# RLHF-V/RLAIF-V

Hardware: NVIDIA B200
Metric: preference-pairs/sec LLaVA-1.5-7B DPO step (higher is better)
Workload: dtype bf16

## Files before the change

### include/rlaifv_b200.h

```cpp
#ifndef RLAIFV_B200_H_
#define RLAIFV_B200_H_

#ifdef __cplusplus
extern "C" {
#endif

const char* rlaifv_last_error(void);

int rlaifv_gemm_bf16(const void* A, long long lda, int a_mn_major, const void* B, long long ldb,
                     int b_mn_major, void* C, long long ldc, int M, int N, int K, const void* bias,
                     const void* residual, long long ldr, int act, int accumulate, int tile_n,
                     void* stream);

int rlaifv_gemm_bf16_scaled(const void* A, long long lda, int a_mn_major, const void* B, long long ldb,
                            int b_mn_major, void* C, long long ldc, int M, int N, int K, const void* bias,
                            const void* residual, long long ldr, int act, int accumulate, int tile_n, float alpha,
                            void* stream);

int rlaifv_gemm_bf16_dual(const void* A, long long lda, int a_mn_major, const void* B, long long ldb, int b_mn_major,
                          const void* A2, long long lda2, const void* B2, long long ldb2, int K2, int r, int n_sub,
                          void* C, long long ldc, int M, int N, int K, const void* bias, const void* residual,
                          long long ldr, int act, int accumulate, void* stream);

int rlaifv_gemm_bf16_swiglu_bwd(const void* A, long long lda, const void* B, long long ldb, int b_mn_major,
// ... 21 lines not shown
                         long long ld_out, const void* d_out, long long ld_dout, const float* lse,
                         float* dq_f32, void* dk, void* dv, long long ld_dkv, float* delta_ws, int nseq,
                         int S, int n_heads, int head_dim, float scale, void* stream);

int rlaifv_attention_fwd_gqa(const void* q, const void* k, const void* v, long long ld_qkv, void* out,
                             long long ld_out, float* lse, int nseq, int S, int n_heads, int n_kv_heads,
                             int head_dim, int causal, float scale, void* stream);
int rlaifv_attention_bwd_gqa(const void* q, const void* k, const void* v, long long ld_qkv, const void* out,
                             long long ld_out, const void* d_out, long long ld_dout, const float* lse, float* dq_f32,
                             void* dk, void* dv, long long ld_dkv, float* delta_ws, int nseq, int S, int n_heads,
                             int n_kv_heads, int head_dim, float scale, void* stream);
int rlaifv_cross_attention_fwd(const void* q, long long ld_q, const void* k, const void* v, long long ld_kv, void* out,
                               long long ld_out, float* lse, int nseq, int Sq, int Skv, int n_heads, int head_dim,
                               int q_shared, float scale, void* stream);
int rlaifv_cross_attention_bwd(const void* q, long long ld_q, const void* k, const void* v, long long ld_kv,
                               const void* out, long long ld_out, const void* d_out, long long ld_dout,
                               const float* lse, float* dq_f32, void* dk, void* dv, long long ld_dkv, float* delta_ws,
                               int nseq, int Sq, int Skv, int n_heads, int head_dim, int q_shared, float scale,
                               void* stream);
int rlaifv_rope_fwd_gqa(void* qkv, const void* cos_tab, const void* sin_tab, long long M, int T, int n_heads,
                        int n_kv_heads, int head_dim, long long ld, void* stream);
int rlaifv_rope_bwd_gqa(void* dqkv, const float* dq_f32, const void* cos_tab, const void* sin_tab, long long M,
                        int T, int n_heads, int n_kv_heads, int head_dim, long long ld, void* stream);

int rlaifv_rmsnorm_fwd(const void* x, const void* w, void* y, float* rstd_or_null, int M, int H, float eps,
                       void* stream);
int rlaifv_rmsnorm_bwd_partials(void);
int rlaifv_rmsnorm_bwd(const void* dy, const void* x, const void* w, const float* rstd,
                       const void* dres_or_null, void* dx, void* dw, int dw_accumulate, float* workspace,
                       int M, int H, void* stream);
int rlaifv_layernorm_fwd(const void* x, const void* w, const void* b, void* y, int M, int H, float eps,
                         void* stream);
int rlaifv_layernorm_bwd(const void* dy, const void* x, const void* w, void* dx, void* dw, void* db, int accumulate,
                         float* workspace, int M, int H, float eps, void* stream);
int rlaifv_add_rows_bcast(const void* x, const void* table, void* y, long long M, int P, int H, void* stream);

int rlaifv_rope_fwd(void* qkv, const void* cos_tab, const void* sin_tab, long long M, int T, int n_heads,
                    int head_dim, long long ld, void* stream);
int rlaifv_rope_bwd(void* dqkv, const float* dq_f32, const void* cos_tab, const void* sin_tab, long long M,
                    int T, int n_heads, int head_dim, long long ld, void* stream);

int rlaifv_swiglu_fwd(const void* gu, void* act, long long M, int F, void* stream);
int rlaifv_swiglu_bwd(const void* gu, const void* dact, void* dgu, long long M, int F, void* stream);
int rlaifv_gelu_fwd(const void* pre, void* post, long long n, void* stream);
int rlaifv_gelu_bwd(const void* pre, const void* dpost, void* dpre, long long n, void* stream);
int rlaifv_colsum(const void* x, long long M, int N, void* db, int accumulate, float* workspace_64xN,
// ... 62 lines not shown
```

### rlaif-v_b200/csrc/rowops.cu

```cuda
#include "common.cuh"
#include "host_util.h"

namespace b200 {

__device__ __forceinline__ void load8(const bf16* p, float (&v)[8]) {
  uint4 u = *reinterpret_cast<const uint4*>(p);
  float2 a = unpack_bf16(u.x), b = unpack_bf16(u.y), c = unpack_bf16(u.z), d = unpack_bf16(u.w);
  v[0] = a.x; v[1] = a.y; v[2] = b.x; v[3] = b.y; v[4] = c.x; v[5] = c.y; v[6] = d.x; v[7] = d.y;
}
__device__ __forceinline__ void store8(bf16* p, const float (&v)[8]) {
  uint4 u;
  u.x = pack_bf16(v[0], v[1]);
  u.y = pack_bf16(v[2], v[3]);
  u.z = pack_bf16(v[4], v[5]);
  u.w = pack_bf16(v[6], v[7]);
  *reinterpret_cast<uint4*>(p) = u;
}

__device__ __forceinline__ float2 block_sum2(float a, float b) {
  __shared__ float sa[32], sb[32];
  a = warp_sum(a);
  b = warp_sum(b);
  const int w = threadIdx.x >> 5, l = threadIdx.x & 31, nw = blockDim.x >> 5;
  __syncthreads();
// ... 334 lines not shown
    const long long row = r / nrot;
    const int pos = (int)(row % T);
    bf16* p = dqkv + row * ld + (long long)head * D + c8 * 8;
    float y1[8], y2[8], c1[8], s1[8], c2[8], s2[8];
    if (head < nh && dq_f32) {
      const float* q = dq_f32 + row * (long long)nh * D + head * D + c8 * 8;
      float4 a = *reinterpret_cast<const float4*>(q), b = *reinterpret_cast<const float4*>(q + 4);
      float4 c = *reinterpret_cast<const float4*>(q + half), d = *reinterpret_cast<const float4*>(q + half + 4);
      y1[0] = a.x; y1[1] = a.y; y1[2] = a.z; y1[3] = a.w; y1[4] = b.x; y1[5] = b.y; y1[6] = b.z; y1[7] = b.w;
      y2[0] = c.x; y2[1] = c.y; y2[2] = c.z; y2[3] = c.w; y2[4] = d.x; y2[5] = d.y; y2[6] = d.z; y2[7] = d.w;
    } else {
      load8(p, y1);
      load8(p + half, y2);
    }
    load8(cosb + (long long)pos * D + c8 * 8, c1);
    load8(sinb + (long long)pos * D + c8 * 8, s1);
    load8(cosb + (long long)pos * D + half + c8 * 8, c2);
    load8(sinb + (long long)pos * D + half + c8 * 8, s2);
    float o1[8], o2[8];
#pragma unroll
    for (int j = 0; j < 8; ++j) {
      o1[j] = y1[j] * c1[j] + y2[j] * s2[j];
      o2[j] = y2[j] * c2[j] - y1[j] * s1[j];
    }
    store8(p, o1);
    store8(p + half, o2);
  }
}

__global__ void swiglu_fwd_kernel(const bf16* __restrict__ gu, bf16* __restrict__ act, long long M,
                                  int F) {
  const int nch = F >> 3;
  const long long total = M * nch;
  const long long T = (long long)gridDim.x * blockDim.x;
  for (long long idx = (long long)blockIdx.x * blockDim.x + threadIdx.x; idx < total; idx += 2 * T) {
    const long long idx2 = idx + T;
    const bool two = idx2 < total;
    const long long row0 = idx / nch, row1 = two ? idx2 / nch : row0;
    const int c0 = (int)(idx - row0 * nch), c1 = two ? (int)(idx2 - row1 * nch) : c0;
    float g0[8], u0[8], g1[8], u1[8], o[8];
    load8(gu + row0 * 2 * F + c0 * 8, g0);
    load8(gu + row0 * 2 * F + F + c0 * 8, u0);
    load8(gu + row1 * 2 * F + c1 * 8, g1);
    load8(gu + row1 * 2 * F + F + c1 * 8, u1);
#pragma unroll
    for (int j = 0; j < 8; ++j) o[j] = bf16_round(g0[j] / (1.f + __expf(-g0[j]))) * u0[j];
// ... 747 lines not shown
  const long long total = M * (n_heads + n_kv_heads) * (head_dim / 16);
  rope_bwd_kernel<<<grid_for(total, 256), 256, 0, ST>>>((bf16*)dqkv, dq_f32, (const bf16*)cos_tab,
                                                        (const bf16*)sin_tab, M, T, n_heads, n_kv_heads, head_dim, ld);
  B200_CHECK_CUDA(cudaGetLastError());
  return 0;
}
extern "C" int rlaifv_rope_fwd(void* qkv, const void* cos_tab, const void* sin_tab, long long M, int T,
                               int n_heads, int head_dim, long long ld, void* stream) {
  return rope_fwd_impl(qkv, cos_tab, sin_tab, M, T, n_heads, n_heads, head_dim, ld, stream);
}
extern "C" int rlaifv_rope_bwd(void* dqkv, const float* dq_f32, const void* cos_tab, const void* sin_tab,
                               long long M, int T, int n_heads, int head_dim, long long ld, void* stream) {
  return rope_bwd_impl(dqkv, dq_f32, cos_tab, sin_tab, M, T, n_heads, n_heads, head_dim, ld, stream);
}
extern "C" int rlaifv_rope_fwd_gqa(void* qkv, const void* cos_tab, const void* sin_tab, long long M, int T,
                                   int n_heads, int n_kv_heads, int head_dim, long long ld, void* stream) {
  return rope_fwd_impl(qkv, cos_tab, sin_tab, M, T, n_heads, n_kv_heads, head_dim, ld, stream);
}
extern "C" int rlaifv_rope_bwd_gqa(void* dqkv, const float* dq_f32, const void* cos_tab, const void* sin_tab,
                                   long long M, int T, int n_heads, int n_kv_heads, int head_dim, long long ld,
                                   void* stream) {
  return rope_bwd_impl(dqkv, dq_f32, cos_tab, sin_tab, M, T, n_heads, n_kv_heads, head_dim, ld, stream);
}

extern "C" int rlaifv_swiglu_fwd(const void* gu, void* act, long long M, int F, void* stream) {
  B200_REQUIRE(F % 8 == 0, "swiglu: F %% 8 != 0");
  swiglu_fwd_kernel<<<grid_for(M * (F / 8), 256), 256, 0, ST>>>((const bf16*)gu, (bf16*)act, M, F);
  B200_CHECK_CUDA(cudaGetLastError());
  return 0;
}
extern "C" int rlaifv_swiglu_bwd(const void* gu, const void* dact, void* dgu, long long M, int F, void* stream) {
  B200_REQUIRE(F % 8 == 0, "swiglu: F %% 8 != 0");
  swiglu_bwd_kernel<<<grid_for(M * (F / 8), 256), 256, 0, ST>>>((const bf16*)gu, (const bf16*)dact, (bf16*)dgu, M, F);
  B200_CHECK_CUDA(cudaGetLastError());
  return 0;
}
extern "C" int rlaifv_gelu_fwd(const void* pre, void* post, long long n, void* stream) {
  B200_REQUIRE(n % 8 == 0, "gelu_fwd: n %% 8 != 0");
  gelu_fwd_kernel<<<grid_for(n / 8, 256), 256, 0, ST>>>((const bf16*)pre, (bf16*)post, n / 8);
  B200_CHECK_CUDA(cudaGetLastError());
  return 0;
}
extern "C" int rlaifv_gelu_bwd(const void* pre, const void* dpost, void* dpre, long long n, void* stream) {
  B200_REQUIRE(n % 8 == 0, "gelu_bwd: n %% 8 != 0");
  gelu_bwd_kernel<<<grid_for(n / 8, 256), 256, 0, ST>>>((const bf16*)pre, (const bf16*)dpost, (bf16*)dpre, n / 8);
  B200_CHECK_CUDA(cudaGetLastError());
// ... 111 lines not shown
  splice_token_weight_kernel<<<grid_for((long long)nseq * (T - 1), 256), 256, 0, ST>>>(src, token_weight, out, nseq, Lw, T);
  B200_CHECK_CUDA(cudaGetLastError());
  return 0;
}
extern "C" int rlaifv_supervised_rows(const long long* labels, int nseq, int T, int cap, int* row_pos, void* stream) {
  B200_REQUIRE(nseq > 0 && T >= 2 && cap > 0, "supervised_rows: bad shape");
  B200_REQUIRE((long long)nseq * T < 2147483647LL, "supervised_rows: nseq*T overflows int32");
  supervised_rows_kernel<<<nseq, 32, 0, ST>>>(labels, nseq, T, cap, row_pos);
  B200_CHECK_CUDA(cudaGetLastError());
  return 0;
}
extern "C" int rlaifv_rows_gather(const int* row_pos, const void* x, void* out, long long n_rows, int H, void* stream) {
  B200_REQUIRE(H % 8 == 0 && n_rows > 0, "rows_gather: bad shape");
  rows_gather_kernel<<<grid_for(n_rows * (H / 8), 256), 256, 0, ST>>>(row_pos, (const bf16*)x, (bf16*)out, n_rows, H / 8);
  B200_CHECK_CUDA(cudaGetLastError());
  return 0;
}
extern "C" int rlaifv_rows_scatter(const int* row_pos, const void* dy, void* dx, long long n_rows, int H, void* stream) {
  B200_REQUIRE(H % 8 == 0 && n_rows > 0, "rows_scatter: bad shape");
  rows_scatter_kernel<<<grid_for(n_rows * (H / 8), 256), 256, 0, ST>>>(row_pos, (const bf16*)dy, (bf16*)dx, n_rows, H / 8);
  B200_CHECK_CUDA(cudaGetLastError());
  return 0;
}
extern "C" int rlaifv_logp_fwd_rows(const void* logits, long long ld, const long long* labels, const int* row_pos,
                                    long long n_rows, int nseq, int T, int V, float* per_tok, float* lse,
                                    float* logp_sum, float* logp_avg, float* count, void* stream) {
  B200_REQUIRE(V % 8 == 0 && T >= 2 && n_rows > 0 && row_pos, "logp_fwd_rows: bad arguments");
  const int grid = (int)(n_rows < (long long)num_sms() * 8 ? n_rows : (long long)num_sms() * 8);
  logp_fwd_kernel<<<grid, LOGP_THREADS, 0, ST>>>((const bf16*)logits, ld, labels, nseq, T, V, per_tok, lse, row_pos,
                                                 n_rows);
  B200_CHECK_CUDA(cudaGetLastError());
  logp_reduce_kernel<<<nseq, 256, 0, ST>>>(per_tok, labels, nseq, T, logp_sum, logp_avg, count);
  B200_CHECK_CUDA(cudaGetLastError());
  return 0;
}
extern "C" int rlaifv_logp_bwd_rows(void* logits, long long ld, const long long* labels, const int* row_pos,
                                    long long n_rows, const float* lse, const float* d_logp, const float* token_weight,
                                    const float* norm, int nseq, int T, int V, void* stream) {
  B200_REQUIRE(V % 8 == 0 && n_rows > 0 && row_pos, "logp_bwd_rows: bad arguments");
  const int grid = (int)(n_rows < (long long)num_sms() * 8 ? n_rows : (long long)num_sms() * 8);
  logp_bwd_weighted_kernel<<<grid, LOGP_THREADS, 0, ST>>>((bf16*)logits, ld, labels, lse, d_logp, token_weight, norm,
                                                          nseq, T, V, row_pos, n_rows);
  B200_CHECK_CUDA(cudaGetLastError());
  return 0;
}
extern "C" int rlaifv_logp_bwd(void* logits, long long ld, const long long* labels, const float* lse,
// ... 81 lines not shown
```

### rlaif-v_b200/lib.py

```python
import ctypes
import os

import torch

_HERE = os.path.dirname(os.path.abspath(__file__))
LIB_PATH = os.path.join(_HERE, "librlaifv_b200.so")

c_void_p = ctypes.c_void_p
c_int = ctypes.c_int
c_ll = ctypes.c_longlong
c_float = ctypes.c_float

_SIGNATURES = {
    "rlaifv_gemm_bf16": [c_void_p, c_ll, c_int, c_void_p, c_ll, c_int, c_void_p, c_ll, c_int, c_int, c_int,
                         c_void_p, c_void_p, c_ll, c_int, c_int, c_int, c_void_p],
    "rlaifv_gemm_bf16_scaled": [c_void_p, c_ll, c_int, c_void_p, c_ll, c_int, c_void_p, c_ll, c_int, c_int, c_int,
                                c_void_p, c_void_p, c_ll, c_int, c_int, c_int, c_float, c_void_p],
    "rlaifv_gemm_bf16_dual": [c_void_p, c_ll, c_int, c_void_p, c_ll, c_int, c_void_p, c_ll, c_void_p, c_ll, c_int, c_int,
                              c_int, c_void_p, c_ll, c_int, c_int, c_int, c_void_p, c_void_p, c_ll, c_int, c_int,
                              c_void_p],
    "rlaifv_gemm_bf16_swiglu_bwd": [c_void_p, c_ll, c_void_p, c_ll, c_int, c_void_p, c_ll, c_void_p, c_ll, c_int, c_void_p,
                                    c_ll, c_void_p, c_ll, c_int, c_int, c_int, c_void_p],
    "rlaifv_gemm_set_2cta": [c_int],
    "rlaifv_attention_set_variant": [c_int],
# ... 12 lines not shown
    "rlaifv_swiglu_fwd": [c_void_p, c_void_p, c_ll, c_int, c_void_p],
    "rlaifv_swiglu_bwd": [c_void_p, c_void_p, c_void_p, c_ll, c_int, c_void_p],
    "rlaifv_gelu_fwd": [c_void_p, c_void_p, c_ll, c_void_p],
    "rlaifv_gelu_bwd": [c_void_p, c_void_p, c_void_p, c_ll, c_void_p],
    "rlaifv_dropout_fwd": [c_void_p, c_void_p, c_ll, c_float, ctypes.c_ulonglong, c_void_p],
    "rlaifv_dropout_bwd_add": [c_void_p, c_void_p, c_ll, c_float, ctypes.c_ulonglong, c_void_p],
    "rlaifv_colsum": [c_void_p, c_ll, c_int, c_void_p, c_int, c_void_p, c_void_p],
    "rlaifv_clip_im2col": [c_void_p, c_void_p, c_int, c_int, c_int, c_int, c_int, c_void_p],
    "rlaifv_clip_embed": [c_void_p, c_void_p, c_void_p, c_void_p, c_int, c_int, c_int, c_void_p],
    "rlaifv_clip_drop_cls": [c_void_p, c_void_p, c_int, c_int, c_int, c_void_p],
    "rlaifv_splice_count": [c_void_p, c_int, c_int, c_int, c_int, c_void_p, c_void_p, c_void_p],
    "rlaifv_splice_map": [c_void_p, c_void_p, c_void_p, c_void_p, c_int, c_int, c_int, c_int, c_int,
                          c_void_p, c_void_p, c_void_p],
    "rlaifv_splice_gather": [c_void_p, c_void_p, c_void_p, c_void_p, c_void_p, c_int, c_int, c_int, c_int,
                             c_void_p],
    "rlaifv_splice_scatter": [c_void_p, c_void_p, c_void_p, c_void_p, c_void_p, c_int, c_int, c_int, c_int,
                              c_void_p],
    "rlaifv_f32_to_bf16": [c_void_p, c_void_p, c_ll, c_int, c_void_p],
    "rlaifv_f32_to_bf16_2d": [c_void_p, c_ll, c_void_p, c_ll, c_ll, c_int, c_int, c_void_p],
    "rlaifv_splice_token_weight": [c_void_p, c_void_p, c_void_p, c_int, c_int, c_int, c_void_p],
    "rlaifv_supervised_rows": [c_void_p, c_int, c_int, c_int, c_void_p, c_void_p],
    "rlaifv_rows_gather": [c_void_p, c_void_p, c_void_p, c_ll, c_int, c_void_p],
    "rlaifv_rows_scatter": [c_void_p, c_void_p, c_void_p, c_ll, c_int, c_void_p],
    "rlaifv_logp_fwd_rows": [c_void_p, c_ll, c_void_p, c_void_p, c_ll, c_int, c_int, c_int, c_void_p, c_void_p, c_void_p,
                             c_void_p, c_void_p, c_void_p],
    "rlaifv_logp_bwd_rows": [c_void_p, c_ll, c_void_p, c_void_p, c_ll, c_void_p, c_void_p, c_void_p, c_void_p, c_int,
                             c_int, c_int, c_void_p],
    "rlaifv_logp_fwd": [c_void_p, c_ll, c_void_p, c_int, c_int, c_int, c_void_p, c_void_p, c_void_p,
                        c_void_p, c_void_p, c_void_p],
    "rlaifv_logp_bwd": [c_void_p, c_ll, c_void_p, c_void_p, c_void_p, c_void_p, c_int, c_int, c_int,
                        c_void_p],
    "rlaifv_dpo_loss": [c_void_p, c_void_p, c_void_p, c_void_p, c_int, c_float, c_float, c_float, c_float,
                        c_void_p, c_void_p, c_void_p, c_void_p, c_void_p, c_void_p, c_void_p],
    "rlaifv_adamw_step": [c_void_p, c_void_p, c_void_p, c_void_p, c_int, c_void_p, c_ll, c_float, c_float,
                          c_float, c_float, c_float, c_int, c_float, c_void_p],
    "rlaifv_attention_fwd_gqa": [c_void_p, c_void_p, c_void_p, c_ll, c_void_p, c_ll, c_void_p, c_int, c_int,
                                 c_int, c_int, c_int, c_int, c_float, c_void_p],
    "rlaifv_attention_bwd_gqa": [c_void_p, c_void_p, c_void_p, c_ll, c_void_p, c_ll, c_void_p, c_ll, c_void_p,
                                 c_void_p, c_void_p, c_void_p, c_ll, c_void_p, c_int, c_int, c_int, c_int, c_int,
                                 c_float, c_void_p],
    "rlaifv_rope_fwd_gqa": [c_void_p, c_void_p, c_void_p, c_ll, c_int, c_int, c_int, c_int, c_ll, c_void_p],
    "rlaifv_rope_bwd_gqa": [c_void_p, c_void_p, c_void_p, c_void_p, c_ll, c_int, c_int, c_int, c_int, c_ll, c_void_p],
    "rlaifv_attention_fwd": [c_void_p, c_void_p, c_void_p, c_ll, c_void_p, c_ll, c_void_p, c_int, c_int,
                             c_int, c_int, c_int, c_float, c_void_p],
    "rlaifv_attention_bwd": [c_void_p, c_void_p, c_void_p, c_ll, c_void_p, c_ll, c_void_p, c_ll, c_void_p,
                             c_void_p, c_void_p, c_void_p, c_ll, c_void_p, c_int, c_int, c_int, c_int,
# ... 117 lines not shown
```

### rlaif-v_b200/model.py

```python
import math
from dataclasses import dataclass, field

import torch

from . import ops

IGNORE_INDEX = -100
IMAGE_TOKEN_INDEX = -200
_BF = torch.bfloat16
_F32 = torch.float32


@dataclass
class LlavaDims:
    vocab_size: int = 32000
    hidden_size: int = 4096
    intermediate_size: int = 11008
    num_layers: int = 32
    num_heads: int = 32
    num_kv_heads: int = 0
    rms_eps: float = 1e-5
    rope_theta: float = 10000.0
    max_len: int = 2048
    clip_hidden: int = 1024
# ... 22 lines not shown
    @property
    def kv_size(self):
        return self.kv_heads * self.head_dim

    @property
    def num_patches(self):
        return (self.image_size // self.patch_size) ** 2

    @property
    def clip_layers_used(self):
        return self.clip_layers + 1 + self.select_layer if self.select_layer < 0 else self.select_layer

    @property
    def patch_k(self):
        return 3 * self.patch_size * self.patch_size

    @property
    def patch_k_pad(self):
        return (self.patch_k + 63) // 64 * 64


def _round_up(n, m):
    return (n + m - 1) // m * m


@dataclass
class Segment:
    name: str
    shape: tuple
    offset: int
    decay: bool


@dataclass
class Bucket:
    name: str
    start: int
    size: int
    decay_size: int
    segments: list = field(default_factory=list)


class ParamStore:
    PAD = 1024

    def __init__(self, dims: LlavaDims, device):
# ... 208 lines not shown
            self.layers.append(L)


class LlavaDPOPolicy:

    def __init__(self, dims: LlavaDims, device="cuda", hf_state=None, seed=0, init_std=0.02):
        self.dims = dims
        self.device = torch.device(device)
        self.store = ParamStore(dims, self.device)
        has_clip = dims.frontend == "clip_mlp"
        if hf_state is not None:
            self.store.load_hf(hf_state)
            self.clip = ClipWeights(dims, self.device, hf_state) if has_clip else None
        else:
            self._random_init(seed, init_std)
            self.clip = ClipWeights(dims, self.device, None, seed + 1) if has_clip else None
        self._rope = {}
        self._bufs = {}
        self.stash_extra = False
        self.stash_act = False
        self.compact_head = True
        self.split_attention_bwd = True
        self.fuse_swiglu_bwd = True
        self.embed_grad_f32 = None
        self._stash = None
        self.lora = None

    def enable_lora(self, r=64, alpha=16, seed=7, init_b_zero=True, dropout=0.0):
        if self.dims.kv_heads != self.dims.num_heads:
            raise NotImplementedError("LoRA adapters on a grouped-query decoder (unequal q/k/v widths)")
        self.lora = LoraStore(self.dims, self.device, r=r, alpha=alpha, seed=seed, init_b_zero=init_b_zero,
                              dropout=dropout)
        return self.lora

    training = True

    def _lora_seed(self, i, group):
        L = self.lora
        g = ("qkv", "o", "gu", "down").index(group)
        return (L.rng_seed * 1000003 + L.step) * 4099 + (self._fwd_count * 131 + i) * 4 + g

    _fwd_count = 0

    def trainable_buckets(self):
        from .zero2 import store_buckets
        if self.lora is None:
# ... 66 lines not shown
            return dx_plain if glu is None else ops.swiglu_bwd(glu, dx_plain, dx_out)
        ops.gemm(dt, x, L.g[f"l{i}.{a_name}"], a_mn=True, b_mn=True, accumulate=acc)
        if glu is not None:
            return ops.gemm_swiglu_bwd(dy, W, glu, dx_out, a2=dt, b2=A)
        return ops.gemm_dual(dy, W, dt, A, dx_out, k2=A.shape[0], r=r, n_sub=0, b_mn=True)

    def _random_init(self, seed, std):
        g = torch.Generator(device=self.device).manual_seed(seed)
        for b in self.store.buckets:
            for s in b.segments:
                v = self.store.p[s.name]
                if len(s.shape) == 1 and (s.name.endswith("ln1") or s.name.endswith("ln2") or s.name == "norm"):
                    v.fill_(1.0)
                elif len(s.shape) == 1:
                    v.zero_()
                else:
                    flat = v.view(-1)
                    step = 1 << 26
                    for o in range(0, flat.numel(), step):
                        n = min(step, flat.numel() - o)
                        flat[o:o + n].copy_(torch.randn(n, generator=g, device=self.device, dtype=_F32) * std)

    def buf(self, key, shape, dtype=_BF):
        t = self._bufs.get(key)
        if t is None or tuple(t.shape) != tuple(shape) or t.dtype != dtype:
            t = torch.empty(shape, dtype=dtype, device=self.device)
            self._bufs[key] = t
        return t

    def rope_tables(self, T):
        if T not in self._rope:
            d = self.dims
            hd = d.head_dim
            inv_freq = 1.0 / (d.rope_theta ** (torch.arange(0, hd, 2, dtype=torch.int64).float() / hd))
            pos = torch.arange(T, dtype=_F32)
            emb = torch.cat([pos[:, None] * inv_freq[None, :]] * 2, dim=-1)
            self._rope[T] = (emb.cos().to(_BF).to(self.device).contiguous(),
                             emb.sin().to(_BF).to(self.device).contiguous())
        return self._rope[T]

    def encode_images(self, images):
        d, cw = self.dims, self.clip
        b = images.shape[0]
        P, C = d.num_patches, d.clip_hidden
        T = P + 1
        img = images.to(device=self.device, dtype=_BF).contiguous()
        cols = ops.clip_im2col(img, d.patch_size, d.patch_k_pad)
        patch = ops.gemm(cols, cw.patch_w)
        x = ops.clip_embed(patch, cw.cls, cw.pos, b, P)
        x = ops.layernorm_fwd(x, cw.pre_ln_w, cw.pre_ln_b, d.clip_eps)
        nh = d.clip_heads
# ... 7 lines not shown
            x2 = ops.gemm(att, L["o_w"], self.buf("clip_x2", x.shape), bias=L["o_b"], residual=x)
            h = ops.layernorm_fwd(x2, L["layer_norm2_w"], L["layer_norm2_b"], d.clip_eps, out=self.buf("clip_h", x.shape))
            f = ops.gemm(h, L["fc1_w"], self.buf("clip_f", (b * T, d.clip_intermediate)), bias=L["fc1_b"],
                         act=ops.ACT_QUICK_GELU)
            x = ops.gemm(f, L["fc2_w"], self.buf("clip_x", x.shape), bias=L["fc2_b"], residual=x2)
        return ops.clip_drop_cls(x, b, P)

    def splice(self, input_ids, labels, image_rows, n_blocks, img_index=None, T_hint=None):
        d = self.dims
        nseq, L = input_ids.shape
        n_img, lens = ops.splice_count(input_ids, d.num_patches, d.max_len)
        if T_hint is None:
            T = int(lens.max().item())
            n_slots = int(torch.clamp(n_img, min=1).sum().item())
        else:
            T, n_slots = T_hint
        if img_index is None:
            img_index = torch.arange(n_slots, dtype=torch.int32, device=self.device)
        src, new_labels = ops.splice_map(input_ids, labels, n_img, img_index, d.num_patches, T, d.max_len)
        embeds = ops.splice_gather(src, input_ids, self.store.p["embed"], image_rows,
                                   out=self.buf("x0", (nseq * T, d.hidden_size)))
        return embeds, new_labels, src, T

    def _run_layers(self, x, nseq, T, st):
        d, P, dev = self.dims, self.store.p, self.device
        H, F, KV = d.hidden_size, d.intermediate_size, d.kv_size
        nh, hd, nkv = d.num_heads, d.head_dim, d.kv_heads
        QKV = H + 2 * KV
        M = nseq * T
        cos, sin = self.rope_tables(T)
        scale = hd ** -0.5
        keep_stash = st is not None
        for i in range(d.num_layers):
            self._need(self.layer_bucket_name(i))
            ls = None
            if keep_stash:
                ls = {"x": x}
                qkv = torch.empty((M, QKV), dtype=_BF, device=dev)
                att = torch.empty((M, H), dtype=_BF, device=dev)
                x2 = torch.empty((M, H), dtype=_BF, device=dev)
                gu = torch.empty((M, 2 * F), dtype=_BF, device=dev)
                x3 = torch.empty((M, H), dtype=_BF, device=dev)
                rstd1 = torch.empty(M, dtype=_F32, device=dev)
                rstd2 = torch.empty(M, dtype=_F32, device=dev)
                lse = torch.empty((nseq, nh, T), dtype=_F32, device=dev)
            else:
                qkv, att = self.buf("qkv", (M, QKV)), self.buf("att", (M, H))
                x2, gu = self.buf("x2", (M, H)), self.buf("gu", (M, 2 * F))
                x3 = self.buf("x3_%d" % (i & 1), (M, H))
                rstd1 = rstd2 = None
                lse = self.buf("lse", (nseq, nh, T), _F32)
            extra = keep_stash and self.stash_extra
            n1 = ops.rmsnorm_fwd(x, P[f"l{i}.ln1"], d.rms_eps,
                                 out=torch.empty((M, H), dtype=_BF, device=dev) if extra else self.buf("n", (M, H)),
                                 rstd=rstd1)
            self._lin_fwd(i, "qkv", n1, qkv, ls=ls if keep_stash else None)
            ops.rope_fwd(qkv, cos, sin, T, nh, hd, n_kv_heads=nkv)
            ops.attention_fwd(qkv[:, :H], qkv[:, H:H + KV], qkv[:, H + KV:], nseq, T, nh, hd, True, scale, out=att,
                              lse=lse, n_kv_heads=nkv)
            self._lin_fwd(i, "o", att, x2, residual=x, ls=ls if keep_stash else None)
            n2 = ops.rmsnorm_fwd(x2, P[f"l{i}.ln2"], d.rms_eps,
                                 out=torch.empty((M, H), dtype=_BF, device=dev) if extra else self.buf("n", (M, H)),
                                 rstd=rstd2)
            self._lin_fwd(i, "gu", n2, gu, ls=ls if keep_stash else None)
            keep_act = extra or (keep_stash and self.stash_act)
            act = ops.swiglu_fwd(gu, torch.empty((M, F), dtype=_BF, device=dev) if keep_act else self.buf("act", (M, F)))
            self._lin_fwd(i, "down", act, x3, residual=x2, ls=ls if keep_stash else None)
            if keep_stash:
                ls.update(qkv=qkv, att=att, x2=x2, gu=gu, rstd1=rstd1, rstd2=rstd2, lse=lse)
                if extra:
                    ls.update(n1=n1, n2=n2, act=act)
                elif keep_act:
                    ls.update(act=act)
                st["layers"].append(ls)
            x = x3
        return x

    def decoder_logits(self, inputs_embeds):
        d = self.dims
        nseq, T, H = inputs_embeds.shape
        x = inputs_embeds.to(device=self.device, dtype=_BF).reshape(nseq * T, H).contiguous()
        x = self._run_layers(x, nseq, T, None)
        self._need("head")
        hn = ops.rmsnorm_fwd(x, self.store.p["norm"], d.rms_eps, out=self.buf("hn", (nseq * T, H)))
        logits = ops.gemm(hn, self.store.p["lm_head"])
        return logits.view(nseq, T, d.vocab_size)

    def forward_logps(self, input_ids, labels, images, keep_stash=True, return_per_token=True, T_hint=None):
        d, P = self.dims, self.store.p
        dev = self.device
        input_ids = input_ids.to(dev).contiguous()
        labels = labels.to(dev).contiguous()
        nseq = input_ids.shape[0]
        b = images.shape[0]
        H, F, V = d.hidden_size, d.intermediate_size, d.vocab_size
        nh, hd = d.num_heads, d.head_dim
        st = {"layers": []} if keep_stash else None
        self._fwd_count += 1

        proj = self._frontend_fwd(images, st)
        n_slots = nseq
        img_index = (torch.arange(n_slots, dtype=torch.int32, device=dev) % b).contiguous() if nseq == 2 * b \
            else torch.arange(n_slots, dtype=torch.int32, device=dev)
        self._need("embed")
        x, new_labels, src, T = self.splice(input_ids, labels, proj, b, img_index,
                                            T_hint=(T_hint, n_slots) if T_hint is not None else None)
        M = nseq * T
        if keep_stash:
            st.update(src=src, input_ids=input_ids, labels=new_labels, T=T, nseq=nseq, b=b,
                      n_feat_rows=proj.shape[0])
        x = self._run_layers(x, nseq, T, st)
        self._need("head")
        compact = keep_stash and self.compact_head
        if compact:
            row_pos = ops.supervised_rows(new_labels, input_ids.shape[1])
            R = row_pos.numel()
            xc = ops.rows_gather(row_pos, x, out=self.buf("xc", (R, H)))
            rstd_f = torch.empty(R, dtype=_F32, device=dev)
            hn = ops.rmsnorm_fwd(xc, P["norm"], d.rms_eps, out=self.buf("hn_c", (R, H)), rstd=rstd_f)
            logits = ops.gemm(hn, P["lm_head"], self.buf("logits_c", (R, V)))
            per_tok, lse_v, logp, avg, count = ops.logp_fwd_rows(logits, new_labels, row_pos, nseq, T)
            st.update(x_final=xc, rstd_f=rstd_f, hn=hn, logits=logits, lse_v=lse_v, count=count, row_pos=row_pos)
            self._stash = st
            return dict(per_token_logps=per_tok, logp=logp, avg_logp=avg, labels=new_labels, T=T)
        rstd_f = torch.empty(M, dtype=_F32, device=dev) if keep_stash else None
        hn = ops.rmsnorm_fwd(x, P["norm"], d.rms_eps, out=self.buf("hn", (M, H)), rstd=rstd_f)
        logits = ops.gemm(hn, P["lm_head"], self.buf("logits", (M, V)))
        per_tok, lse_v, logp, avg, count = ops.logp_fwd(logits, new_labels, nseq, T)
        if keep_stash:
            st.update(x_final=x, rstd_f=rstd_f, hn=hn, logits=logits, lse_v=lse_v, count=count)
            self._stash = st
        return dict(per_token_logps=per_tok, logp=logp, avg_logp=avg, labels=new_labels, T=T)

    def backward_logps(self, d_logp, use_average=False, accumulate=False, token_weight=None, weight_sum=None):
        st = self._stash
        assert st is not None, "forward_logps(keep_stash=True) must precede backward_logps"
# ... 15 lines not shown
            dlogits = ops.logp_bwd_rows(st["logits"], st["labels"], row_pos, st["lse_v"], d_logp, nseq, T,
                                        token_weight=token_weight, norm=norm)
        elif token_weight is not None:
            dlogits = ops.logp_bwd_weighted(st["logits"], st["labels"], st["lse_v"], d_logp, token_weight, nseq, T,
                                            wsum=weight_sum if use_average else None)
        else:
            dlogits = ops.logp_bwd(st["logits"], st["labels"], st["lse_v"], d_logp, nseq, T,
                                   count=st["count"] if use_average else None)
        frozen = self.lora is not None
        scratch_h = self.buf("frozen_dw", (H,)) if frozen else None
        Mh = dlogits.shape[0]
        if not frozen:
            ops.gemm(dlogits, st["hn"], G["lm_head"], a_mn=True, b_mn=True, accumulate=acc)
        dhn = ops.gemm(dlogits, P["lm_head"], self.buf("dn_c" if row_pos is not None else "dn", (Mh, H)), b_mn=True)
        dx = ops.rmsnorm_bwd(dhn, st["x_final"], P["norm"], st["rstd_f"],
                             self.buf("dx_c" if row_pos is not None else "dx_a", (Mh, H)),
                             scratch_h if frozen else G["norm"], dw_accumulate=acc and not frozen)
        if row_pos is not None:
            full = self.buf("dx_a", (M, H))
            full.zero_()
            dx = ops.rows_scatter(row_pos, dx, full)
        if self.on_head_grads_ready is not None:
            self.on_head_grads_ready()
        for i in reversed(range(d.num_layers)):
            ls = st["layers"][i]
            act = ls["act"] if "act" in ls else ops.swiglu_fwd(ls["gu"], self.buf("act", (M, F)))
            if self.fuse_swiglu_bwd and F % 64 == 0:
                dgu = self._lin_bwd(i, "down", dx, act, self.buf("dgu", (M, 2 * F)), ls, acc, glu=ls["gu"])
            else:
                dact = self._lin_bwd(i, "down", dx, act, self.buf("dact", (M, F)), ls, acc)
                dgu = ops.swiglu_bwd(ls["gu"], dact, self.buf("dgu", (M, 2 * F)))
            n2 = ls["n2"] if "n2" in ls else ops.rmsnorm_fwd(ls["x2"], P[f"l{i}.ln2"], d.rms_eps,
                                                             out=self.buf("n", (M, H)))
            dn2 = self._lin_bwd(i, "gu", dgu, n2, self.buf("dn", (M, H)), ls, acc)
            dx2 = ops.rmsnorm_bwd(dn2, ls["x2"], P[f"l{i}.ln2"], ls["rstd2"], self.buf("dx_b", (M, H)),
                                  scratch_h if frozen else G[f"l{i}.ln2"], dres=dx, dw_accumulate=acc and not frozen)
            datt = self._lin_bwd(i, "o", dx2, ls["att"], self.buf("datt", (M, H)), ls, acc)
            qkv = ls["qkv"]
            dqkv = self.buf("dqkv", (M, H + 2 * KV))
            if self.split_attention_bwd:
                ops.attention_bwd_split(qkv[:, :H], qkv[:, H:H + KV], qkv[:, H + KV:], ls["att"], datt, ls["lse"], nseq,
                                        T, T, nh, hd, True, scale, dqkv[:, :H], dqkv[:, H:H + KV], dqkv[:, H + KV:],
                                        n_kv_heads=nkv, delta_ws=self.buf("delta", (nseq, nh, T), _F32))
                ops.rope_bwd(dqkv, None, cos, sin, T, nh, hd, n_kv_heads=nkv)
            else:
                dq32 = self.buf("dq32", (M, H), _F32)
                dq32.zero_()
                ops.attention_bwd(qkv[:, :H], qkv[:, H:H + KV], qkv[:, H + KV:], ls["att"], datt, ls["lse"], nseq, T, nh,
# ... 62 lines not shown
```

### rlaif-v_b200/omnilmm_model.py

```python
import torch

from . import ops
from .model import LlavaDims, LlavaDPOPolicy
from .resampler import Resampler

_BF = torch.bfloat16


def omnilmm_dims(**kw):
    base = dict(frontend="resampler", hidden_size=4096, intermediate_size=14336, num_layers=32, num_heads=32,
                num_kv_heads=8, rms_eps=1e-5, rope_theta=10000.0, vocab_size=32008, num_query=64, vision_width=1792,
                im_patch_token=32000, im_start_token=32001, im_end_token=32002)
    base.update(kw)
    return LlavaDims(**base)


class OmniLMMDPOPolicy(LlavaDPOPolicy):
    def __init__(self, dims: LlavaDims, device="cuda", hf_state=None, seed=0, init_std=0.02, eva_dims=None):
        assert dims.frontend == "resampler" and dims.hidden_size % 128 == 0
        assert min(dims.im_patch_token, dims.im_start_token, dims.im_end_token) >= 0, "set the <im_*> token ids"
        super().__init__(dims, device, hf_state=hf_state, seed=seed, init_std=init_std)
        grid = int(round(dims.num_query ** 0.5))
        assert grid * grid == dims.num_query
        pre = "model.resampler."
        rstate = None if hf_state is None else {k[len(pre):]: v for k, v in hf_state.items() if k.startswith(pre)}
        self.resampler = Resampler(grid, dims.hidden_size, dims.hidden_size // 128, dims.vision_width, self.device,
                                   state=rstate, seed=seed + 2)
        self.vision_token_grad = None
        self.tower = None
        if eva_dims is not None:
            from .eva_tower import EvaTower
            assert eva_dims.embed_dim == dims.vision_width
            tpre = "model.vision_tower."
            tstate = None if hf_state is None else {k[len(tpre):]: v for k, v in hf_state.items() if k.startswith(tpre)}
            self.tower = EvaTower(eva_dims, self.device, state=tstate or None, seed=seed + 3)
            self.tower.param_ready = self._need
            self.tower.on_block_grads_ready = self._tower_block_ready

    on_bucket_grads_ready = None

    def _tower_block_ready(self, i):
        if self.on_bucket_grads_ready is not None:
            self.on_bucket_grads_ready("eva_embed" if i == "embed" else "eva%d" % i)

# ... 64 lines not shown
```

### rlaif-v_b200/ops.py

```python
import torch

from . import lib as _l

ACT_NONE, ACT_GELU, ACT_QUICK_GELU = 0, 1, 2
IGNORE_INDEX = -100
IMAGE_TOKEN_INDEX = -200


def _chk(t, dtype=torch.bfloat16):
    assert t.is_cuda and t.dtype == dtype, (t.device, t.dtype)
    return t


def gemm(a, b, out=None, *, a_mn=False, b_mn=False, bias=None, residual=None, act=ACT_NONE,
         accumulate=False, tile_n=0, alpha=1.0):
    _chk(a), _chk(b)
    assert a.dim() == 2 and b.dim() == 2 and a.stride(1) == 1 and b.stride(1) == 1
    if a_mn:
        K, M = a.shape
    else:
        M, K = a.shape
    if b_mn:
        Kb, N = b.shape
    else:
# ... 156 lines not shown
    if out is None:
        out = torch.empty_like(x)
    _l.call("rlaifv_add_rows_bcast", _l.ptr(x), _l.ptr(table), _l.ptr(out), x.shape[0], table.shape[0], x.shape[1],
            _l.stream_ptr())
    return out


def rope_fwd(qkv, cos, sin, T, n_heads, head_dim, n_kv_heads=None):
    _chk(qkv), _chk(cos), _chk(sin)
    _l.call("rlaifv_rope_fwd_gqa", _l.ptr(qkv), _l.ptr(cos), _l.ptr(sin), qkv.shape[0], T, n_heads,
            n_heads if n_kv_heads is None else n_kv_heads, head_dim, qkv.stride(0), _l.stream_ptr())
    return qkv


def rope_bwd(dqkv, dq_f32, cos, sin, T, n_heads, head_dim, n_kv_heads=None):
    _chk(dqkv)
    if dq_f32 is not None:
        _chk(dq_f32, _f32)
    _l.call("rlaifv_rope_bwd_gqa", _l.ptr(dqkv), _l.ptr(dq_f32), _l.ptr(cos), _l.ptr(sin), dqkv.shape[0], T,
            n_heads, n_heads if n_kv_heads is None else n_kv_heads, head_dim, dqkv.stride(0), _l.stream_ptr())
    return dqkv


def swiglu_fwd(gu, out=None):
    _chk(gu)
    M, F2 = gu.shape
    if out is None:
        out = torch.empty((M, F2 // 2), dtype=torch.bfloat16, device=gu.device)
    _l.call("rlaifv_swiglu_fwd", _l.ptr(gu), _l.ptr(out), M, F2 // 2, _l.stream_ptr())
    return out


def swiglu_bwd(gu, dact, dgu=None):
    _chk(gu), _chk(dact)
    M, F2 = gu.shape
    if dgu is None:
        dgu = torch.empty_like(gu)
    _l.call("rlaifv_swiglu_bwd", _l.ptr(gu), _l.ptr(dact), _l.ptr(dgu), M, F2 // 2, _l.stream_ptr())
    return dgu


def gelu_fwd(pre, post=None):
    _chk(pre)
    if post is None:
        post = torch.empty_like(pre)
    _l.call("rlaifv_gelu_fwd", _l.ptr(pre), _l.ptr(post), pre.numel(), _l.stream_ptr())
# ... 134 lines not shown
    _chk(labels, torch.int64)
    assert labels.is_contiguous()
    nseq, T = labels.shape
    row_pos = torch.empty(nseq * cap, dtype=torch.int32, device=labels.device)
    _l.call("rlaifv_supervised_rows", _l.ptr(labels), nseq, T, int(cap), _l.ptr(row_pos), _l.stream_ptr())
    return row_pos


def rows_gather(row_pos, x, out=None):
    _chk(x)
    assert x.is_contiguous() and row_pos.dtype == torch.int32
    n, H = row_pos.numel(), x.shape[1]
    if out is None:
        out = torch.empty((n, H), dtype=torch.bfloat16, device=x.device)
    _l.call("rlaifv_rows_gather", _l.ptr(row_pos), _l.ptr(x), _l.ptr(out), n, H, _l.stream_ptr())
    return out


def rows_scatter(row_pos, dy, dx):
    _chk(dy), _chk(dx)
    assert dy.is_contiguous() and dx.is_contiguous() and dy.shape[1] == dx.shape[1]
    _l.call("rlaifv_rows_scatter", _l.ptr(row_pos), _l.ptr(dy), _l.ptr(dx), row_pos.numel(), dy.shape[1], _l.stream_ptr())
    return dx


def logp_fwd_rows(logits, labels, row_pos, nseq, T):
    _chk(logits)
    V, dev, n = logits.shape[1], logits.device, row_pos.numel()
    assert logits.shape[0] == n
    per_tok = torch.zeros((nseq, T - 1), dtype=_f32, device=dev)
    lse = torch.zeros(n, dtype=_f32, device=dev)
    s = torch.empty(nseq, dtype=_f32, device=dev)
    a = torch.empty(nseq, dtype=_f32, device=dev)
    c = torch.empty(nseq, dtype=_f32, device=dev)
    _l.call("rlaifv_logp_fwd_rows", _l.ptr(logits), logits.stride(0), _l.ptr(labels), _l.ptr(row_pos), n, nseq, T, V,
            _l.ptr(per_tok), _l.ptr(lse), _l.ptr(s), _l.ptr(a), _l.ptr(c), _l.stream_ptr())
    return per_tok, lse, s, a, c


def logp_bwd_rows(logits, labels, row_pos, lse, d_logp, nseq, T, token_weight=None, norm=None):
    _chk(logits), _chk(lse, _f32), _chk(d_logp, _f32)
    _l.call("rlaifv_logp_bwd_rows", _l.ptr(logits), logits.stride(0), _l.ptr(labels), _l.ptr(row_pos), row_pos.numel(),
            _l.ptr(lse), _l.ptr(d_logp), _l.ptr(token_weight), _l.ptr(norm), nseq, T, logits.shape[1], _l.stream_ptr())
    return logits


# ... 99 lines not shown
```

Before: 11.70.

## Share common chosen/rejected prefix rows in decoder forward via dedup maps

Computes the token positions where the chosen and rejected sequences of a DPO pair share an identical prefix, then runs the per-row layer work (norms, QKV, o-proj, MLP) on a deduplicated row set. A new fused kernel applies RoPE while expanding QKV back to full rows for attention, and attention output is gathered back to deduplicated rows. The backward pass expands the stashed activations to full rows and recomputes the norms. This adds gathers, a host sync for the prefix count and recompute in backward, and any gain depends on how long the shared prefixes are.

```diff
diff --git a/include/rlaifv_b200.h b/include/rlaifv_b200.h
--- a/include/rlaifv_b200.h
+++ b/include/rlaifv_b200.h
@@ -67,6 +67,9 @@
                         int n_kv_heads, int head_dim, long long ld, void* stream);
 int rlaifv_rope_bwd_gqa(void* dqkv, const float* dq_f32, const void* cos_tab, const void* sin_tab, long long M,
                         int T, int n_heads, int n_kv_heads, int head_dim, long long ld, void* stream);
+int rlaifv_rope_fwd_expand(const void* qkv_d, long long ld_d, const int* f2d, const void* cos_tab, const void* sin_tab,
+                           void* qkv, long long ld, long long M, int T, int n_heads, int n_kv_heads, int head_dim,
+                           void* stream);
 
 int rlaifv_rmsnorm_fwd(const void* x, const void* w, void* y, float* rstd_or_null, int M, int H, float eps,
                        void* stream);
diff --git a/rlaif-v_b200/csrc/rowops.cu b/rlaif-v_b200/csrc/rowops.cu
--- a/rlaif-v_b200/csrc/rowops.cu
+++ b/rlaif-v_b200/csrc/rowops.cu
@@ -380,6 +380,46 @@
     for (int j = 0; j < 8; ++j) {
       o1[j] = y1[j] * c1[j] + y2[j] * s2[j];
       o2[j] = y2[j] * c2[j] - y1[j] * s1[j];
+    }
+    store8(p, o1);
+    store8(p + half, o2);
+  }
+}
+
+__global__ void rope_fwd_expand_kernel(const bf16* __restrict__ qkv_d, const int* __restrict__ f2d,
+                                       const bf16* __restrict__ cosb, const bf16* __restrict__ sinb,
+                                       bf16* __restrict__ qkv, long long M, int T, int nrot, int nall, int D,
+                                       long long ld_d, long long ld) {
+  const int half = D >> 1;
+  const int per_head = half >> 3;
+  const long long total = M * nall * per_head;
+  for (long long idx = (long long)blockIdx.x * blockDim.x + threadIdx.x; idx < total;
+       idx += (long long)gridDim.x * blockDim.x) {
+    const int c8 = (int)(idx % per_head);
+    long long r = idx / per_head;
+    const int head = (int)(r % nall);
+    const long long row = r / nall;
+    const long long col = (long long)head * D + c8 * 8;
+    const bf16* s = qkv_d + (long long)f2d[row] * ld_d + col;
+    bf16* p = qkv + row * ld + col;
+    if (head >= nrot) {
+      *reinterpret_cast<uint4*>(p) = *reinterpret_cast<const uint4*>(s);
+      *reinterpret_cast<uint4*>(p + half) = *reinterpret_cast<const uint4*>(s + half);
+      continue;
+    }
+    const int pos = (int)(row % T);
+    float x1[8], x2[8], c1[8], s1[8], c2[8], s2[8];
+    load8(s, x1);
+    load8(s + half, x2);
+    load8(cosb + (long long)pos * D + c8 * 8, c1);
+    load8(sinb + (long long)pos * D + c8 * 8, s1);
+    load8(cosb + (long long)pos * D + half + c8 * 8, c2);
+    load8(sinb + (long long)pos * D + half + c8 * 8, s2);
+    float o1[8], o2[8];
+#pragma unroll
+    for (int j = 0; j < 8; ++j) {
+      o1[j] = bf16_round(x1[j] * c1[j]) + bf16_round(-x2[j] * s1[j]);
+      o2[j] = bf16_round(x2[j] * c2[j]) + bf16_round(x1[j] * s2[j]);
     }
     store8(p, o1);
     store8(p + half, o2);
@@ -1173,6 +1213,17 @@
                                    void* stream) {
   return rope_bwd_impl(dqkv, dq_f32, cos_tab, sin_tab, M, T, n_heads, n_kv_heads, head_dim, ld, stream);
 }
+extern "C" int rlaifv_rope_fwd_expand(const void* qkv_d, long long ld_d, const int* f2d, const void* cos_tab,
+                                      const void* sin_tab, void* qkv, long long ld, long long M, int T, int n_heads,
+                                      int n_kv_heads, int head_dim, void* stream) {
+  B200_REQUIRE(head_dim % 16 == 0 && M > 0 && ld_d % 8 == 0 && ld % 8 == 0, "rope_fwd_expand: bad shape");
+  const int nrot = n_heads + n_kv_heads, nall = n_heads + 2 * n_kv_heads;
+  rope_fwd_expand_kernel<<<grid_for(M * nall * (head_dim / 16), 256), 256, 0, ST>>>(
+      (const bf16*)qkv_d, f2d, (const bf16*)cos_tab, (const bf16*)sin_tab, (bf16*)qkv, M, T, nrot, nall, head_dim,
+      ld_d, ld);
+  B200_CHECK_CUDA(cudaGetLastError());
+  return 0;
+}
 
 extern "C" int rlaifv_swiglu_fwd(const void* gu, void* act, long long M, int F, void* stream) {
   B200_REQUIRE(F % 8 == 0, "swiglu: F %% 8 != 0");
@@ -1330,6 +1381,7 @@
   B200_CHECK_CUDA(cudaGetLastError());
   return 0;
 }
+
 extern "C" int rlaifv_logp_fwd_rows(const void* logits, long long ld, const long long* labels, const int* row_pos,
                                     long long n_rows, int nseq, int T, int V, float* per_tok, float* lse,
                                     float* logp_sum, float* logp_avg, float* count, void* stream) {
diff --git a/rlaif-v_b200/lib.py b/rlaif-v_b200/lib.py
--- a/rlaif-v_b200/lib.py
+++ b/rlaif-v_b200/lib.py
@@ -58,6 +58,8 @@
     "rlaifv_supervised_rows": [c_void_p, c_int, c_int, c_int, c_void_p, c_void_p],
     "rlaifv_rows_gather": [c_void_p, c_void_p, c_void_p, c_ll, c_int, c_void_p],
     "rlaifv_rows_scatter": [c_void_p, c_void_p, c_void_p, c_ll, c_int, c_void_p],
+    "rlaifv_rope_fwd_expand": [c_void_p, c_ll, c_void_p, c_void_p, c_void_p, c_void_p, c_ll, c_ll, c_int, c_int, c_int,
+                               c_int, c_void_p],
     "rlaifv_logp_fwd_rows": [c_void_p, c_ll, c_void_p, c_void_p, c_ll, c_int, c_int, c_int, c_void_p, c_void_p, c_void_p,
                              c_void_p, c_void_p, c_void_p],
     "rlaifv_logp_bwd_rows": [c_void_p, c_ll, c_void_p, c_void_p, c_ll, c_void_p, c_void_p, c_void_p, c_void_p, c_int,
diff --git a/rlaif-v_b200/model.py b/rlaif-v_b200/model.py
--- a/rlaif-v_b200/model.py
+++ b/rlaif-v_b200/model.py
@@ -1,4 +1,5 @@
 import math
+import os
 from dataclasses import dataclass, field
 
 import torch
@@ -68,6 +69,45 @@
 
 def _round_up(n, m):
     return (n + m - 1) // m * m
+
+
+@dataclass
+class PrefixShare:
+    m_d: int
+    d2f: torch.Tensor
+    twin: torch.Tensor
+    f2d_copy: torch.Tensor
+    f2d_grad: torch.Tensor
+
+
+def prefix_share_maps(src, input_ids, b, T):
+    dev = src.device
+    s = src.long()
+    tok = torch.gather(input_ids, 1, s.clamp(min=0))
+    key = torch.where(s >= 0, tok, s - 1)
+    P = (key[:b] == key[b:]).long().cumprod(1).sum(1)
+    n_twin = int(P.sum().item())
+    if n_twin == 0:
+        return None
+    bT = b * T
+    m_d = 2 * bT - n_twin
+    t = torch.arange(T, device=dev)[None, :]
+    i = torch.arange(b, device=dev)[:, None]
+    is_twin = t < P[:, None]
+    L_rej = T - P
+    off = bT + torch.cumsum(L_rej, 0) - L_rej
+    win = torch.arange(bT, device=dev)
+    rej_copy = torch.where(is_twin, i * T + t, off[:, None] + t - P[:, None]).reshape(-1)
+    is_twin = is_twin.reshape(-1)
+    f2d_copy = torch.cat([win, rej_copy])
+    f2d_grad = torch.cat([win, torch.where(is_twin, -1, rej_copy)])
+    d2f = torch.empty(m_d + 1, dtype=torch.long, device=dev)
+    d2f[:bT] = win
+    d2f.scatter_(0, torch.where(is_twin, m_d, rej_copy), bT + win)
+    twin = torch.full((m_d,), -1, dtype=torch.long, device=dev)
+    twin[:bT] = torch.where(is_twin, bT + win, -1)
+    i32 = torch.int32
+    return PrefixShare(m_d, d2f[:m_d].to(i32).contiguous(), twin.to(i32), f2d_copy.to(i32), f2d_grad.to(i32))
 
 
 @dataclass
@@ -322,6 +362,7 @@
         self.compact_head = True
         self.split_attention_bwd = True
         self.fuse_swiglu_bwd = True
+        self.share_prefix = os.environ.get("RLAIFV_SHARE_PREFIX", "1") != "0"
         self.embed_grad_f32 = None
         self._stash = None
         self.lora = None
@@ -434,11 +475,12 @@
                         flat[o:o + n].copy_(torch.randn(n, generator=g, device=self.device, dtype=_F32) * std)
 
     def buf(self, key, shape, dtype=_BF):
+        n = math.prod(shape)
         t = self._bufs.get(key)
-        if t is None or tuple(t.shape) != tuple(shape) or t.dtype != dtype:
-            t = torch.empty(shape, dtype=dtype, device=self.device)
+        if t is None or t.numel() < n or t.dtype != dtype:
+            t = torch.empty(n, dtype=dtype, device=self.device)
             self._bufs[key] = t
-        return t
+        return t[:n].view(shape)
 
     def rope_tables(self, T):
         if T not in self._rope:
@@ -492,12 +534,13 @@
                                    out=self.buf("x0", (nseq * T, d.hidden_size)))
         return embeds, new_labels, src, T
 
-    def _run_layers(self, x, nseq, T, st):
+    def _run_layers(self, x, nseq, T, st, sp=None):
         d, P, dev = self.dims, self.store.p, self.device
         H, F, KV = d.hidden_size, d.intermediate_size, d.kv_size
         nh, hd, nkv = d.num_heads, d.head_dim, d.kv_heads
         QKV = H + 2 * KV
         M = nseq * T
+        Mr = M if sp is None else sp.m_d
         cos, sin = self.rope_tables(T)
         scale = hd ** -0.5
         keep_stash = st is not None
@@ -507,44 +550,66 @@
             if keep_stash:
                 ls = {"x": x}
                 qkv = torch.empty((M, QKV), dtype=_BF, device=dev)
-                att = torch.empty((M, H), dtype=_BF, device=dev)
-                x2 = torch.empty((M, H), dtype=_BF, device=dev)
-                gu = torch.empty((M, 2 * F), dtype=_BF, device=dev)
-                x3 = torch.empty((M, H), dtype=_BF, device=dev)
-                rstd1 = torch.empty(M, dtype=_F32, device=dev)
-                rstd2 = torch.empty(M, dtype=_F32, device=dev)
+                att = torch.empty((Mr, H), dtype=_BF, device=dev)
+                x2 = torch.empty((Mr, H), dtype=_BF, device=dev)
+                gu = torch.empty((Mr, 2 * F), dtype=_BF, device=dev)
+                x3 = torch.empty((Mr, H), dtype=_BF, device=dev)
+                rstd1 = torch.empty(M, dtype=_F32, device=dev) if sp is None else None
+                rstd2 = torch.empty(M, dtype=_F32, device=dev) if sp is None else None
                 lse = torch.empty((nseq, nh, T), dtype=_F32, device=dev)
             else:
-                qkv, att = self.buf("qkv", (M, QKV)), self.buf("att", (M, H))
-                x2, gu = self.buf("x2", (M, H)), self.buf("gu", (M, 2 * F))
-                x3 = self.buf("x3_%d" % (i & 1), (M, H))
+                qkv, att = self.buf("qkv", (M, QKV)), self.buf("att", (Mr, H))
+                x2, gu = self.buf("x2", (Mr, H)), self.buf("gu", (Mr, 2 * F))
+                x3 = self.buf("x3_%d" % (i & 1), (Mr, H))
                 rstd1 = rstd2 = None
                 lse = self.buf("lse", (nseq, nh, T), _F32)
             extra = keep_stash and self.stash_extra
+            keep_n = extra and sp is None
             n1 = ops.rmsnorm_fwd(x, P[f"l{i}.ln1"], d.rms_eps,
-                                 out=torch.empty((M, H), dtype=_BF, device=dev) if extra else self.buf("n", (M, H)),
+                                 out=torch.empty((Mr, H), dtype=_BF, device=dev) if keep_n else self.buf("n", (Mr, H)),
                                  rstd=rstd1)
-            self._lin_fwd(i, "qkv", n1, qkv, ls=ls if keep_stash else None)
-            ops.rope_fwd(qkv, cos, sin, T, nh, hd, n_kv_heads=nkv)
-            ops.attention_fwd(qkv[:, :H], qkv[:, H:H + KV], qkv[:, H + KV:], nseq, T, nh, hd, True, scale, out=att,
+            if sp is None:
+                self._lin_fwd(i, "qkv", n1, qkv, ls=ls if keep_stash else None)
+                ops.rope_fwd(qkv, cos, sin, T, nh, hd, n_kv_heads=nkv)
+                att_f = att
+            else:
+                qkv_d = self._lin_fwd(i, "qkv", n1, self.buf("qkv_d", (Mr, QKV)), ls=ls if keep_stash else None)
+                ops.rope_fwd_expand(qkv_d, sp.f2d_copy, cos, sin, T, nh, hd, qkv, n_kv_heads=nkv)
+                att_f = self.buf("att_f", (M, H))
+            ops.attention_fwd(qkv[:, :H], qkv[:, H:H + KV], qkv[:, H + KV:], nseq, T, nh, hd, True, scale, out=att_f,
                               lse=lse, n_kv_heads=nkv)
+            if sp is not None:
+                ops.rows_gather(sp.d2f, att_f, out=att)
             self._lin_fwd(i, "o", att, x2, residual=x, ls=ls if keep_stash else None)
             n2 = ops.rmsnorm_fwd(x2, P[f"l{i}.ln2"], d.rms_eps,
-                                 out=torch.empty((M, H), dtype=_BF, device=dev) if extra else self.buf("n", (M, H)),
+                                 out=torch.empty((Mr, H), dtype=_BF, device=dev) if keep_n else self.buf("n", (Mr, H)),
                                  rstd=rstd2)
             self._lin_fwd(i, "gu", n2, gu, ls=ls if keep_stash else None)
             keep_act = extra or (keep_stash and self.stash_act)
-            act = ops.swiglu_fwd(gu, torch.empty((M, F), dtype=_BF, device=dev) if keep_act else self.buf("act", (M, F)))
+            act = ops.swiglu_fwd(gu, torch.empty((Mr, F), dtype=_BF, device=dev) if keep_act else self.buf("act", (Mr, F)))
             self._lin_fwd(i, "down", act, x3, residual=x2, ls=ls if keep_stash else None)
             if keep_stash:
                 ls.update(qkv=qkv, att=att, x2=x2, gu=gu, rstd1=rstd1, rstd2=rstd2, lse=lse)
-                if extra:
+                if keep_n:
                     ls.update(n1=n1, n2=n2, act=act)
                 elif keep_act:
                     ls.update(act=act)
                 st["layers"].append(ls)
             x = x3
         return x
+
+    def _expand_stash(self, i, ls, sp, M):
+        d, P = self.dims, self.store.p
+        full = {k: v for k, v in ls.items() if k in ("qkv", "lse") or k.startswith("seed_")}
+        for k, v in ls.items():
+            if k in ("x", "x2", "gu", "act", "att") or k.startswith("t_"):
+                full[k] = ops.rows_gather(sp.f2d_copy, v, out=self.buf("full_" + k, (M, v.shape[1])))
+        for j, src in (("1", "x"), ("2", "x2")):
+            rstd = self.buf("full_rstd" + j, (M,), _F32)
+            full["n" + j] = ops.rmsnorm_fwd(full[src], P[f"l{i}.ln{j}"], d.rms_eps,
+                                            out=self.buf("full_n" + j, (M, d.hidden_size)), rstd=rstd)
+            full["rstd" + j] = rstd
+        return full
 
     def decoder_logits(self, inputs_embeds):
         d = self.dims
@@ -555,6 +620,12 @@
         hn = ops.rmsnorm_fwd(x, self.store.p["norm"], d.rms_eps, out=self.buf("hn", (nseq * T, H)))
         logits = ops.gemm(hn, self.store.p["lm_head"])
         return logits.view(nseq, T, d.vocab_size)
+
+    def _share_prefix_on(self, nseq, b, keep_stash):
+        if not self.share_prefix or nseq != 2 * b or not self.split_attention_bwd:
+            return False
+        L = self.lora
+        return not (L is not None and L.dropout > 0.0 and self.training and keep_stash)
 
     def forward_logps(self, input_ids, labels, images, keep_stash=True, return_per_token=True, T_hint=None):
         d, P = self.dims, self.store.p
@@ -576,12 +647,20 @@
         x, new_labels, src, T = self.splice(input_ids, labels, proj, b, img_index,
                                             T_hint=(T_hint, n_slots) if T_hint is not None else None)
         M = nseq * T
+        sp = None
+        if self._share_prefix_on(nseq, b, keep_stash):
+            sp = prefix_share_maps(src, input_ids, b, T)
+            if sp is not None:
+                x = ops.rows_gather(sp.d2f, x, out=self.buf("x0_d", (sp.m_d, H)))
         if keep_stash:
             st.update(src=src, input_ids=input_ids, labels=new_labels, T=T, nseq=nseq, b=b,
-                      n_feat_rows=proj.shape[0])
-        x = self._run_layers(x, nseq, T, st)
+                      n_feat_rows=proj.shape[0], sp=sp)
+        x = self._run_layers(x, nseq, T, st, sp)
         self._need("head")
         compact = keep_stash and self.compact_head
+        if sp is not None:
+            x = ops.rows_gather(sp.f2d_copy, x, out=self.buf("x_full", (M, H)) if compact or not keep_stash
+                                else torch.empty((M, H), dtype=_BF, device=dev))
         if compact:
             row_pos = ops.supervised_rows(new_labels, input_ids.shape[1])
             R = row_pos.numel()
@@ -643,8 +722,11 @@
             dx = ops.rows_scatter(row_pos, dx, full)
         if self.on_head_grads_ready is not None:
             self.on_head_grads_ready()
+        sp = st.get("sp")
         for i in reversed(range(d.num_layers)):
             ls = st["layers"][i]
+            if sp is not None:
+                ls = self._expand_stash(i, ls, sp, M)
             act = ls["act"] if "act" in ls else ops.swiglu_fwd(ls["gu"], self.buf("act", (M, F)))
             if self.fuse_swiglu_bwd and F % 64 == 0:
                 dgu = self._lin_bwd(i, "down", dx, act, self.buf("dgu", (M, 2 * F)), ls, acc, glu=ls["gu"])
diff --git a/rlaif-v_b200/omnilmm_model.py b/rlaif-v_b200/omnilmm_model.py
--- a/rlaif-v_b200/omnilmm_model.py
+++ b/rlaif-v_b200/omnilmm_model.py
@@ -20,6 +20,7 @@
         assert dims.frontend == "resampler" and dims.hidden_size % 128 == 0
         assert min(dims.im_patch_token, dims.im_start_token, dims.im_end_token) >= 0, "set the <im_*> token ids"
         super().__init__(dims, device, hf_state=hf_state, seed=seed, init_std=init_std)
+        self.share_prefix = False
         grid = int(round(dims.num_query ** 0.5))
         assert grid * grid == dims.num_query
         pre = "model.resampler."
diff --git a/rlaif-v_b200/ops.py b/rlaif-v_b200/ops.py
--- a/rlaif-v_b200/ops.py
+++ b/rlaif-v_b200/ops.py
@@ -202,6 +202,15 @@
     return dqkv
 
 
+def rope_fwd_expand(qkv_d, f2d, cos, sin, T, n_heads, head_dim, out, n_kv_heads=None):
+    _chk(qkv_d), _chk(cos), _chk(sin), _chk(out)
+    assert f2d.dtype == torch.int32 and out.shape[0] == f2d.numel() and qkv_d.stride(1) == 1 and out.stride(1) == 1
+    _l.call("rlaifv_rope_fwd_expand", _l.ptr(qkv_d), qkv_d.stride(0), _l.ptr(f2d), _l.ptr(cos), _l.ptr(sin),
+            _l.ptr(out), out.stride(0), out.shape[0], T, n_heads, n_heads if n_kv_heads is None else n_kv_heads,
+            head_dim, _l.stream_ptr())
+    return out
+
+
 def swiglu_fwd(gu, out=None):
     _chk(gu)
     M, F2 = gu.shape
@@ -382,6 +391,7 @@
     assert dy.is_contiguous() and dx.is_contiguous() and dy.shape[1] == dx.shape[1]
     _l.call("rlaifv_rows_scatter", _l.ptr(row_pos), _l.ptr(dy), _l.ptr(dx), row_pos.numel(), dy.shape[1], _l.stream_ptr())
     return dx
+
 
 
 def logp_fwd_rows(logits, labels, row_pos, nseq, T):
```

New measurement: 12.34 (median of 6 runs). 1.05x the previous value.
